# JunFenngZhi/YOLO-Fastest-and-Embedded-deployment

Hardware: AMD Instinct MI355X
Metric: frames/sec end-to-end (model forward + decode + per-class NMS), 320x256 batch=256 per GPU (higher is better)
Workload: dtype f32; 1 GPU; YOLO-Fastest 320x256 batch=256 fp32 per GPU, synthetic uniform-u8 frames (BASELINE.json configs[1]); global_batch=256, weights=yolo_fastest_256x320_epoch28.pth, kmax=64, chunk=0, in_flight=2, lanes=1, branches=0, world_size=1, parallelism=single GPU

## Files before the change

### yolo-fastest-and-embedded-deployment_amd/csrc/yf_mres_kernels.hip

```cpp
#include <hip/hip_runtime.h>
#include <math.h>
#include <stdint.h>

#include "yf_kernels.h"


namespace yf {



typedef float f32x4 __attribute__((ext_vector_type(4)));
typedef float f32x2 __attribute__((ext_vector_type(2)));
__device__ __forceinline__ float relu_bits(float x) { return __int_as_float(max(__float_as_int(x), 0)); }

template <int NT2>
__device__ __forceinline__ void mres_project_f32(float (&d)[4], const float (&w2f)[4][NT2], f32x4 (&acc)[NT2])
{
#pragma unroll
    for (int j = 0; j < 4; ++j) d[j] = relu_bits(d[j]);
    __builtin_amdgcn_sched_barrier(0);
#pragma unroll
    for (int j = 0; j < 4; ++j)
#pragma unroll
        for (int nt = 0; nt < NT2; ++nt) acc[nt] = __builtin_amdgcn_mfma_f32_16x16x4f32(w2f[j][nt], d[j], acc[nt], 0, 0, 0);
}

__host__ __device__ constexpr int mres_epl(int mtr, int s = 1) { return mtr * 16 + (s == 2 ? 1 : 0); }
__host__ __device__ constexpr int mres_ksteps(int K) { return (K / 16) * 4 + ((K % 16) ? 2 : 0); }
__host__ __device__ constexpr int mres_chunk_floats(int cin, int cout, int wmode = WM_F32)
{
    return wmode != WM_F32 ? (wmode == WM_F16X3 ? 2 : 1) * ((mres_ksteps(cin) + 3) / 4) * 128 + 16 + 9 * 16 + 16 +
                                 (wmode == WM_F16X3 ? 2 : 1) * ((cout + 15) / 16) * 128
                           : mres_ksteps(cin) * 64 + 16 + 9 * 16 + 16 + 4 * ((cout + 15) / 16) * 64;
}

template <int CIN, int S, int RW, int NRP, int MTR, int XP, int WFLOATS, int NTHR, typename T>
__device__ __forceinline__ void mres_stage(const MresArgs& a, int n, int oy0, int ox0, float* X, float* WL)
{
    constexpr int C4 = CIN / 4, NX = MTR * 16 * C4, NXI = (NX + NTHR - 1) / NTHR, NW4 = WFLOATS / 4, NWI = (NW4 + NTHR - 1) / NTHR;
    const T* __restrict__ src = reinterpret_cast<const T*>(a.in) + (long)n * a.H * a.W * CIN;
    float4 wv[NWI], xv[NXI];
#pragma unroll
    for (int i = 0; i < NWI; ++i) {
        const int idx = threadIdx.x + i * NTHR;
        wv[i] = float4(*reinterpret_cast<const float4*>(a.wp + 4 * (idx < NW4 ? idx : NW4 - 1)));
    }
#pragma unroll
    for (int i = 0; i < NXI; ++i) {
        const int idx = threadIdx.x + i * NTHR;
        const int rp = idx / C4, c4 = idx - rp * C4;
        const int ry = rp / RW, rx = rp - ry * RW;
        const int iy = oy0 * S - 1 + ry, ix = ox0 * S - 1 + rx;
        const bool ok = rp < NRP && iy >= 0 && iy < a.H && ix >= 0 && ix < a.W;
        xv[i] = ld4<T>(src + (ok ? (iy * a.W + ix) * CIN + c4 * 4 : 0));
        if (!ok) xv[i] = make_float4(0.f, 0.f, 0.f, 0.f);
    }
#pragma unroll
    for (int i = 0; i < NWI; ++i) {
        const int idx = threadIdx.x + i * NTHR;
        if (idx < NW4) *reinterpret_cast<float4*>(&WL[4 * idx]) = wv[i];
    }
#pragma unroll
    for (int i = 0; i < NXI; ++i) {
        const int idx = threadIdx.x + i * NTHR;
        const int rp = idx / C4, c4 = idx - rp * C4;
        if (idx < NX) *reinterpret_cast<float4*>(&X[rp * XP + c4 * 4]) = xv[i];
    }
}

__host__ __device__ constexpr bool mres_writes_expansion(int cin, int cexp, int cout, int s) { return cin == 24 && cexp == 136 && cout == 48 && s == 2; }
__host__ __device__ constexpr bool mres_relu_out(int cin, int cexp, int cout, int s) { return mres_writes_expansion(cin, cexp, cout, s); }

template <int TH, int TW, int RW, int S>
__device__ __forceinline__ void mres_out_px(int mo, int r, int& oy, int& ox)
{
    if constexpr (S == 1 && RW % 16 == 6 && TW % 2 == 0 && TH % 8 == 0) {
        const int rb = mo / (TW / 2), cp = mo - rb * (TW / 2);
        oy = rb * 8 + (r >> 1);
        ox = cp * 2 + (r & 1);
    } else if constexpr (S == 1 && RW % 16 == 12 && TW == 10 && TH == 8) {
        if (mo < 4) { oy = (mo >> 1) * 4 + (r >> 2); ox = (mo & 1) * 4 + (r & 3); }
        else { oy = r >> 1; ox = 8 + (r & 1); }
    } else {
        const int op = mo * 16 + r;
        oy = op / TW;
        ox = op - oy * TW;
    }
}

template <int CIN, int CEXP, int COUT, bool RES, int S, int TH, int TW, int NWAVE, typename T>
__global__ void __launch_bounds__(NWAVE * 64) mres_kernel(MresArgs a)
{
    constexpr int RH = (TH - 1) * S + 3, RW = (TW - 1) * S + 3, NRP = RH * RW;
    constexpr int MTR = (NRP + 15) / 16, MTO = (TH * TW) / 16;
    constexpr int MTRW = (MTR + NWAVE - 1) / NWAVE, MTOW = (MTO + NWAVE - 1) / NWAVE;
    constexpr bool EVEN_R = MTR % NWAVE == 0, EVEN_O = MTO % NWAVE == 0;
    constexpr bool WEXP = mres_writes_expansion(CIN, CEXP, COUT, S);
    constexpr int XP = CIN + 4;
    constexpr int EPL = mres_epl(MTR, S);
    constexpr bool X3 = is_x3<T>::value;
    constexpr bool H16 = sizeof(T) == 2 || X3;
    constexpr int WM = X3 ? 2 : 1;
    constexpr int KS1 = mres_ksteps(CIN), NB1 = CIN / 16, NT2 = (COUT + 15) / 16, NCH = (CEXP + 15) / 16;
    constexpr int NK1 = (KS1 + 3) / 4;
    constexpr int OFF_B1 = H16 ? WM * NK1 * 128 : KS1 * 64, OFF_WD = OFF_B1 + 16, OFF_BD = OFF_WD + 144, OFF_W2 = OFF_BD + 16;
    constexpr int CHUNK = OFF_W2 + (H16 ? WM * NT2 * 128 : 4 * NT2 * 64);
    static_assert((TH * TW) % 16 == 0 && CIN % 8 == 0 && COUT % 4 == 0, "shape");
    static_assert(!RES || (CIN == COUT && S == 1), "residual needs same shape");
    static_assert(CHUNK == mres_chunk_floats(CIN, COUT, wmode_of<T>()), "pack layout");
    static_assert(MTRW <= 32, "in-image mask bits");
    extern __shared__ __attribute__((aligned(16))) float mres_smem[];
    float* X = mres_smem;
    float* E = mres_smem + MTR * 16 * XP;
    float* WL = E + 16 * EPL;
    constexpr int WFLOATS = (NCH * CHUNK + COUT + 3) & ~3;

    const int b = xcd_tile(blockIdx.x, gridDim.x);
    const int tx = b % a.tiles_x, ty = (b / a.tiles_x) % a.tiles_y, n = b / (a.tiles_x * a.tiles_y);
    const int oy0 = ty * TH, ox0 = tx * TW;
    const int Ho = a.H / S, Wo = a.W / S;
    const int wave = __builtin_amdgcn_readfirstlane((int)(threadIdx.x >> 6));
    const int lane = threadIdx.x & 63, r = lane & 15, q = lane >> 4;

    mres_stage<CIN, S, RW, NRP, MTR, XP, WFLOATS, NWAVE * 64, T>(a, n, oy0, ox0, X, WL);
    __syncthreads();

    float a1[MTRW][KS1];
    unsigned inmask = 0;
    int eoff[MTRW];
#pragma unroll
    for (int i = 0; i < MTRW; ++i) {
        const int mt = wave + i * NWAVE;
        const int row = (mt < MTR ? mt : 0) * 16 + r;
#pragma unroll
        for (int kb = 0; kb < NB1; ++kb) {
            const float4 t = *reinterpret_cast<const float4*>(&X[row * XP + kb * 16 + 4 * q]);
            a1[i][kb * 4 + 0] = t.x; a1[i][kb * 4 + 1] = t.y; a1[i][kb * 4 + 2] = t.z; a1[i][kb * 4 + 3] = t.w;
        }
        if constexpr (CIN % 16 != 0) {
            const float2 t = *reinterpret_cast<const float2*>(&X[row * XP + NB1 * 16 + 2 * q]);
            a1[i][NB1 * 4 + 0] = t.x; a1[i][NB1 * 4 + 1] = t.y;
        }
        {
            const int rp = mt * 16 + r;
            const int ry = rp / RW, rx = rp - ry * RW;
            const int iy = oy0 * S - 1 + ry, ix = ox0 * S - 1 + rx;
            if (mt < MTR && rp < NRP && iy >= 0 && iy < a.H && ix >= 0 && ix < a.W) inmask |= 1u << i;
            eoff[i] = (inmask >> i & 1) && ry > 0 && rx > 0 ? (iy * a.W + ix) * CEXP + 4 * q : -1;
        }
    }
    f16x4 a1h[X3 ? MTRW : 1][NK1], a1l[X3 ? MTRW : 1][NK1];
    if constexpr (X3) {
#pragma unroll
        for (int i = 0; i < MTRW; ++i)
#pragma unroll
            for (int s = 0; s < NK1; ++s)
                split_f16x4(a1[i][4 * s], a1[i][4 * s + 1], 4 * s + 2 < KS1 ? a1[i][(4 * s + 2) % KS1] : 0.f,
                            4 * s + 3 < KS1 ? a1[i][(4 * s + 3) % KS1] : 0.f, a1h[i][s], a1l[i][s]);
    }
    f32x4 acc[MTOW][NT2];
    int rp0[MTOW];
#pragma unroll
    for (int i = 0; i < MTOW; ++i) {
#pragma unroll
        for (int nt = 0; nt < NT2; ++nt) acc[i][nt] = f32x4{0.f, 0.f, 0.f, 0.f};
        const int mo = wave + i * NWAVE;
        int oy, ox;
        mres_out_px<TH, TW, RW, S>(mo < MTO ? mo : 0, r, oy, ox);
        rp0[i] = (oy * S + 1) * RW + ox * S + 1;
    }

#pragma unroll 1
    for (int c = 0; c < NCH; ++c) {
        const float* wc = WL + c * CHUNK;
        float w1f[KS1];
        f16x4 w1h[NK1], w1l[X3 ? NK1 : 1];
        if constexpr (H16) {
#pragma unroll
            for (int s = 0; s < NK1; ++s) w1h[s] = reinterpret_cast<const f16x4*>(wc)[s * 64 + lane];
            if constexpr (X3) {
#pragma unroll
                for (int s = 0; s < NK1; ++s) w1l[s] = reinterpret_cast<const f16x4*>(wc)[(NK1 + s) * 64 + lane];
            }
        } else {
#pragma unroll
            for (int s = 0; s < KS1; ++s) w1f[s] = wc[s * 64 + lane];
        }
        const float4 b1 = *reinterpret_cast<const float4*>(wc + OFF_B1 + 4 * q);
        float4 wd[9];
#pragma unroll
        for (int t = 0; t < 9; ++t) wd[t] = *reinterpret_cast<const float4*>(wc + OFF_WD + t * 16 + 4 * q);
        const float4 bd = *reinterpret_cast<const float4*>(wc + OFF_BD + 4 * q);
        float w2f[4][NT2];
        f16x4 w2h[NT2], w2l[X3 ? NT2 : 1];
        if constexpr (H16) {
#pragma unroll
            for (int nt = 0; nt < NT2; ++nt) w2h[nt] = reinterpret_cast<const f16x4*>(wc + OFF_W2)[nt * 64 + lane];
            if constexpr (X3) {
#pragma unroll
                for (int nt = 0; nt < NT2; ++nt) w2l[nt] = reinterpret_cast<const f16x4*>(wc + OFF_W2)[(NT2 + nt) * 64 + lane];
            }
        } else {
#pragma unroll
            for (int j = 0; j < 4; ++j)
#pragma unroll
                for (int nt = 0; nt < NT2; ++nt) w2f[j][nt] = wc[OFF_W2 + (j * NT2 + nt) * 64 + lane];
        }

#pragma unroll
        for (int i = 0; i < MTRW; ++i) {
            const int mt = wave + i * NWAVE;
            if (EVEN_R || i < MTRW - 1 || mt < MTR) {
                f32x4 cf = f32x4{b1.x, b1.y, b1.z, b1.w};
                if constexpr (X3) {
#pragma unroll
                    for (int s = 0; s < NK1; ++s) {
                        cf = __builtin_amdgcn_mfma_f32_16x16x16f16(w1l[s], a1h[i][s], cf, 0, 0, 0);
                        cf = __builtin_amdgcn_mfma_f32_16x16x16f16(w1h[s], a1l[i][s], cf, 0, 0, 0);
                    }
#pragma unroll
                    for (int s = 0; s < NK1; ++s) cf = __builtin_amdgcn_mfma_f32_16x16x16f16(w1h[s], a1h[i][s], cf, 0, 0, 0);
                } else if constexpr (H16) {
#pragma unroll
                    for (int s = 0; s < NK1; ++s) {
                        const f16x4 ah = f16x4{(half_t)a1[i][4 * s], (half_t)a1[i][4 * s + 1], 4 * s + 2 < KS1 ? (half_t)a1[i][(4 * s + 2) % KS1] : (half_t)0.f,
                                               4 * s + 3 < KS1 ? (half_t)a1[i][(4 * s + 3) % KS1] : (half_t)0.f};
                        cf = __builtin_amdgcn_mfma_f32_16x16x16f16(w1h[s], ah, cf, 0, 0, 0);
                    }
                } else {
#pragma unroll
                    for (int s = 0; s < KS1; ++s) cf = __builtin_amdgcn_mfma_f32_16x16x4f32(w1f[s], a1[i][s], cf, 0, 0, 0);
                }
                const float lim = (inmask >> i) & 1 ? __builtin_inff() : 0.f;
                const float4 ev = make_float4(__builtin_amdgcn_fmed3f(cf[0], 0.f, lim), __builtin_amdgcn_fmed3f(cf[1], 0.f, lim),
                                              __builtin_amdgcn_fmed3f(cf[2], 0.f, lim), __builtin_amdgcn_fmed3f(cf[3], 0.f, lim));
                *reinterpret_cast<float4*>(E + (q * EPL + mt * 16 + r) * 4) = ev;
                if constexpr (WEXP)
                    if (eoff[i] >= 0 && c * 16 + 4 * q < CEXP)
                        st4<T>(reinterpret_cast<T*>(a.out_exp) + (long)n * a.H * a.W * CEXP + eoff[i] + c * 16, ev);
            }
        }
        __syncthreads();
#pragma unroll
        for (int i = 0; i < MTOW; ++i) {
            const int mo = wave + i * NWAVE;
            if (EVEN_O || i < MTOW - 1 || mo < MTO) {
                const float4* e = reinterpret_cast<const float4*>(E) + q * EPL + rp0[i];
                float d[4] = {bd.x, bd.y, bd.z, bd.w};
                constexpr bool BATCH9 = CEXP > 32;
                float4 v9[9];
                if constexpr (BATCH9) {
#pragma unroll
                    for (int t = 0; t < 9; ++t) v9[t] = e[(t / 3 - 1) * RW + (t % 3 - 1)];
                    __builtin_amdgcn_sched_barrier(0);
                }
                f32x2 dl = {d[0], d[1]}, dh2 = {d[2], d[3]};
#pragma unroll
                for (int t = 0; t < 9; ++t) {
                    float4 v;
                    if constexpr (BATCH9) v = v9[t]; else v = e[(t / 3 - 1) * RW + (t % 3 - 1)];
                    const float4 w = wd[t];
                    dl = __builtin_elementwise_fma(f32x2{v.x, v.y}, f32x2{w.x, w.y}, dl);
                    dh2 = __builtin_elementwise_fma(f32x2{v.z, v.w}, f32x2{w.z, w.w}, dh2);
                }
                d[0] = dl[0]; d[1] = dl[1]; d[2] = dh2[0]; d[3] = dh2[1];
                if constexpr (X3) {
                    f16x4 dh, dl;
                    split_f16x4(relu_bits(d[0]), relu_bits(d[1]), relu_bits(d[2]), relu_bits(d[3]), dh, dl);
#pragma unroll
                    for (int nt = 0; nt < NT2; ++nt) acc[i][nt] = __builtin_amdgcn_mfma_f32_16x16x16f16(w2l[nt], dh, acc[i][nt], 0, 0, 0);
#pragma unroll
                    for (int nt = 0; nt < NT2; ++nt) acc[i][nt] = __builtin_amdgcn_mfma_f32_16x16x16f16(w2h[nt], dl, acc[i][nt], 0, 0, 0);
#pragma unroll
                    for (int nt = 0; nt < NT2; ++nt) acc[i][nt] = __builtin_amdgcn_mfma_f32_16x16x16f16(w2h[nt], dh, acc[i][nt], 0, 0, 0);
                } else if constexpr (H16) {
                    const f16x4 dh = f16x4{(half_t)fmaxf(d[0], 0.f), (half_t)fmaxf(d[1], 0.f), (half_t)fmaxf(d[2], 0.f), (half_t)fmaxf(d[3], 0.f)};
#pragma unroll
                    for (int nt = 0; nt < NT2; ++nt) acc[i][nt] = __builtin_amdgcn_mfma_f32_16x16x16f16(w2h[nt], dh, acc[i][nt], 0, 0, 0);
                } else {
                    mres_project_f32<NT2>(d, w2f, acc[i]);
                }
            }
        }
        __syncthreads();
    }

    const float* b2 = WL + NCH * CHUNK;
#pragma unroll
    for (int i = 0; i < MTOW; ++i) {
        const int mo = wave + i * NWAVE;
        if (!EVEN_O && i == MTOW - 1 && mo >= MTO) continue;
        int oy, ox;
        mres_out_px<TH, TW, RW, S>(mo, r, oy, ox);
        const int gy = oy0 + oy, gx = ox0 + ox;
        if (gy >= Ho || gx >= Wo) continue;
#pragma unroll
        for (int nt = 0; nt < NT2; ++nt) {
            const int col = nt * 16 + 4 * q;
            if (col >= COUT) continue;
            const float4 bias = *reinterpret_cast<const float4*>(b2 + col);
            float4 v = make_float4(acc[i][nt][0] + bias.x, acc[i][nt][1] + bias.y, acc[i][nt][2] + bias.z, acc[i][nt][3] + bias.w);
            if constexpr (RES) {
                const float4 x = *reinterpret_cast<const float4*>(&X[((oy + 1) * RW + ox + 1) * XP + col]);
                v.x += x.x; v.y += x.y; v.z += x.z; v.w += x.w;
            }
            if constexpr (mres_relu_out(CIN, CEXP, COUT, S)) v = make_float4(fmaxf(v.x, 0.f), fmaxf(v.y, 0.f), fmaxf(v.z, 0.f), fmaxf(v.w, 0.f));
            st4<T>(reinterpret_cast<T*>(a.out) + (((long)n * Ho + gy) * Wo + gx) * COUT + col, v);
        }
    }
}


template <int K, int NOUT>
struct MresPostFrag { float w[mres_ksteps(K)]; float4 bias; };

template <int K, int NOUT, int NWAVE>
__device__ __forceinline__ void mres_post_fetch(const float* __restrict__ pw, int wave, int lane, MresPostFrag<K, NOUT>& f)
{
    constexpr int KS = mres_ksteps(K), NT = NOUT / 16;
    static_assert(K % 16 == 0 && NOUT % 16 == 0 && NWAVE >= NT, "post conv shape");
    const int nt = wave % NT;
#pragma unroll
    for (int s = 0; s < KS; ++s) f.w[s] = pw[(s * NT + nt) * 64 + lane];
    f.bias = *reinterpret_cast<const float4*>(pw + KS * NT * 64 + nt * 16 + 4 * (lane >> 4));
}

template <int K, int NOUT, int TH, int TW, int RW, int XP, int NWAVE, typename T>
__device__ __forceinline__ void mres_post_conv(const float* X, const MresPostFrag<K, NOUT>& f, T* __restrict__ out, int wave, int lane,
                                               int n, int oy0, int ox0, int H, int W)
{
    constexpr int NB = K / 16, NT = NOUT / 16, MTO = (TH * TW) / 16, NG = NWAVE / NT;
    const int r = lane & 15, q = lane >> 4;
    const int nt = wave % NT, g = wave / NT;
    if (g >= NG) return;
#pragma unroll 1
    for (int mt = g; mt < MTO; mt += NG) {
        const int p = mt * 16 + r, oy = p / TW, ox = p - oy * TW;
        const float* xr = X + ((oy + 1) * RW + ox + 1) * XP + 4 * q;
        float4 av[NB];
#pragma unroll
        for (int kb = 0; kb < NB; ++kb) av[kb] = *reinterpret_cast<const float4*>(xr + kb * 16);
        f32x4 acc = f32x4{0.f, 0.f, 0.f, 0.f};
#pragma unroll
        for (int kb = 0; kb < NB; ++kb)
#pragma unroll
            for (int j = 0; j < 4; ++j) acc = __builtin_amdgcn_mfma_f32_16x16x4f32(f.w[kb * 4 + j], ((const float*)&av[kb])[j], acc, 0, 0, 0);
        const int gy = oy0 + oy, gx = ox0 + ox;
        if (gy >= H || gx >= W) continue;
        const float4 v = make_float4(fmaxf(acc[0] + f.bias.x, 0.f), fmaxf(acc[1] + f.bias.y, 0.f), fmaxf(acc[2] + f.bias.z, 0.f),
                                     fmaxf(acc[3] + f.bias.w, 0.f));
        st4<T>(out + (((long)n * H + gy) * W + gx) * NOUT + nt * 16 + 4 * q, v);
    }
}

template <int CIN, int CEXP, int COUT, bool RES, int TH, int TW, int NWP, int NWC, typename T, int POSTN = 0, bool FRAME = false, int CPP = 1>
__global__ void __launch_bounds__((NWP + NWC) * 64) mres_pc_kernel(MresArgs a)
{
    constexpr int NWAVE = NWP + NWC;
    constexpr int RH = TH + 2, RW = TW + 2, NRP = RH * RW;
    constexpr int MTR = (NRP + 15) / 16, MTO = (TH * TW) / 16;
    constexpr int MTP = FRAME ? MTO : MTR;
    constexpr int MTRW = (MTP + NWP - 1) / NWP, MTOW = (MTO + NWC - 1) / NWC;
    constexpr int XP = CIN + 4;
    constexpr int EPL = mres_epl(MTR);
    constexpr bool X3 = is_x3<T>::value;
    constexpr bool H16 = sizeof(T) == 2 || X3;
    constexpr int WM = X3 ? 2 : 1;
    constexpr int KS1 = mres_ksteps(CIN), NB1 = CIN / 16, NT2 = (COUT + 15) / 16, NCH = (CEXP + 15) / 16;
    constexpr int NK1 = (KS1 + 3) / 4;
    constexpr int OFF_B1 = H16 ? WM * NK1 * 128 : KS1 * 64, OFF_WD = OFF_B1 + 16, OFF_BD = OFF_WD + 144, OFF_W2 = OFF_BD + 16;
    constexpr int CHUNK = OFF_W2 + (H16 ? WM * NT2 * 128 : 4 * NT2 * 64);
    static_assert((TH * TW) % 16 == 0 && CIN % 8 == 0 && COUT % 4 == 0, "shape");
    static_assert(CHUNK == mres_chunk_floats(CIN, COUT, wmode_of<T>()), "pack layout");
    static_assert(!RES || CIN == COUT, "residual needs same shape");
    static_assert(MTRW * 4 <= 64, "in-image mask bits");
    extern __shared__ __attribute__((aligned(16))) float mres_smem[];
    float* X = mres_smem;
    float* E = mres_smem + MTR * 16 * XP;
    float* WL = E + 2 * CPP * 16 * EPL;
    constexpr int NPH = ((CEXP + 15) / 16) / CPP;
    static_assert(((CEXP + 15) / 16) % CPP == 0, "chunks per phase must divide the chunk count");
    constexpr int WFLOATS = (NCH * CHUNK + COUT + 3) & ~3;
    constexpr bool PSUM = !H16 && CIN == 48 && CEXP == 224 && COUT == 48;

    const int b = xcd_tile(blockIdx.x, gridDim.x);
    const int tx = b % a.tiles_x, ty = (b / a.tiles_x) % a.tiles_y, n = b / (a.tiles_x * a.tiles_y);
    const int oy0 = ty * TH, ox0 = tx * TW;
    const int wave = __builtin_amdgcn_readfirstlane((int)(threadIdx.x >> 6));
    const int lane = threadIdx.x & 63, r = lane & 15, q = lane >> 4;
// ... 134 lines not shown
            mres_out_px<TH, TW, RW, 1>(mo < MTO ? mo : 0, r, oy, ox);
            rp0[i] = (oy + 1) * RW + ox + 1;
        }
#pragma unroll 1
      for (int blk = 0; blk < nblk; ++blk) {
        f32x4 acc[MTOW][NT2];
#pragma unroll
        for (int i = 0; i < MTOW; ++i)
#pragma unroll
            for (int nt = 0; nt < NT2; ++nt) acc[i][nt] = f32x4{0.f, 0.f, 0.f, 0.f};
#pragma unroll 1
        for (int ph = 0; ph <= NPH; ++ph) {
#pragma unroll
            for (int u = 0; u < CPP; ++u)
            if (ph >= 1) {
                const int s1 = (ph - 1) * CPP + u;
                const float* wc = WL + s1 * CHUNK;
                const float* Eb = E + (((ph - 1) & 1) * CPP + u) * 16 * EPL;
                float4 wd[9];
#pragma unroll
                for (int t = 0; t < 9; ++t) wd[t] = *reinterpret_cast<const float4*>(wc + OFF_WD + t * 16 + 4 * q);
                const float4 bd = *reinterpret_cast<const float4*>(wc + OFF_BD + 4 * q);
                float w2f[4][NT2];
                f16x4 w2h[NT2], w2l[X3 ? NT2 : 1];
                if constexpr (H16) {
#pragma unroll
                    for (int nt = 0; nt < NT2; ++nt) w2h[nt] = reinterpret_cast<const f16x4*>(wc + OFF_W2)[nt * 64 + lane];
                    if constexpr (X3) {
#pragma unroll
                        for (int nt = 0; nt < NT2; ++nt) w2l[nt] = reinterpret_cast<const f16x4*>(wc + OFF_W2)[(NT2 + nt) * 64 + lane];
                    }
                } else {
#pragma unroll
                    for (int j = 0; j < 4; ++j)
#pragma unroll
                        for (int nt = 0; nt < NT2; ++nt) w2f[j][nt] = wc[OFF_W2 + (j * NT2 + nt) * 64 + lane];
                }
#pragma unroll
                for (int i = 0; i < MTOW; ++i) {
                    const int mo = cw + i * NWC;
                    if (i < MTOW - 1 || mo < MTO) {
                        const float4* e = reinterpret_cast<const float4*>(Eb) + q * EPL + rp0[i];
                        float d[4] = {bd.x, bd.y, bd.z, bd.w};
                        float4 v9[9];
#pragma unroll
                        for (int t = 0; t < 9; ++t) v9[t] = e[(t / 3 - 1) * RW + (t % 3 - 1)];
                        __builtin_amdgcn_sched_barrier(0);
                        f32x2 dl = {d[0], d[1]}, dh2 = {d[2], d[3]};
#pragma unroll
                        for (int t = 0; t < 9; ++t) {
                            const float4 v = v9[t], w = wd[t];
                            dl = __builtin_elementwise_fma(f32x2{v.x, v.y}, f32x2{w.x, w.y}, dl);
                            dh2 = __builtin_elementwise_fma(f32x2{v.z, v.w}, f32x2{w.z, w.w}, dh2);
                        }
                        d[0] = dl[0]; d[1] = dl[1]; d[2] = dh2[0]; d[3] = dh2[1];
                        if constexpr (X3) {
                            f16x4 dh, dl;
                            split_f16x4(relu_bits(d[0]), relu_bits(d[1]), relu_bits(d[2]), relu_bits(d[3]), dh, dl);
#pragma unroll
                            for (int nt = 0; nt < NT2; ++nt) acc[i][nt] = __builtin_amdgcn_mfma_f32_16x16x16f16(w2l[nt], dh, acc[i][nt], 0, 0, 0);
#pragma unroll
                            for (int nt = 0; nt < NT2; ++nt) acc[i][nt] = __builtin_amdgcn_mfma_f32_16x16x16f16(w2h[nt], dl, acc[i][nt], 0, 0, 0);
#pragma unroll
                            for (int nt = 0; nt < NT2; ++nt) acc[i][nt] = __builtin_amdgcn_mfma_f32_16x16x16f16(w2h[nt], dh, acc[i][nt], 0, 0, 0);
                        } else if constexpr (H16) {
                            const f16x4 dh = f16x4{(half_t)fmaxf(d[0], 0.f), (half_t)fmaxf(d[1], 0.f), (half_t)fmaxf(d[2], 0.f),
                                                   (half_t)fmaxf(d[3], 0.f)};
#pragma unroll
                            for (int nt = 0; nt < NT2; ++nt)
                                acc[i][nt] = __builtin_amdgcn_mfma_f32_16x16x16f16(w2h[nt], dh, acc[i][nt], 0, 0, 0);
                        } else if constexpr (PSUM) {
                            f32x4 part[NT2];
#pragma unroll
                            for (int nt = 0; nt < NT2; ++nt) part[nt] = f32x4{0.f, 0.f, 0.f, 0.f};
                            mres_project_f32<NT2>(d, w2f, part);
#pragma unroll
                            for (int nt = 0; nt < NT2; ++nt) acc[i][nt] += part[nt];
                        } else {
                            mres_project_f32<NT2>(d, w2f, acc[i]);
                        }
                    }
                }
            }
            __syncthreads();
        }
        const bool last = blk + 1 == nblk;
        const float* b2 = WL + NCH * CHUNK;
#pragma unroll
        for (int i = 0; i < MTOW; ++i) {
            const int mo = cw + i * NWC;
            if (i == MTOW - 1 && mo >= MTO) continue;
            int oy, ox;
            mres_out_px<TH, TW, RW, 1>(mo, r, oy, ox);
            const int gy = oy0 + oy, gx = ox0 + ox;
            if (gy >= a.H || gx >= a.W) continue;
#pragma unroll
            for (int nt = 0; nt < NT2; ++nt) {
                const int col = nt * 16 + 4 * q;
                if (col >= COUT) continue;
                const float4 bias = *reinterpret_cast<const float4*>(b2 + col);
                float4 v = make_float4(acc[i][nt][0] + bias.x, acc[i][nt][1] + bias.y, acc[i][nt][2] + bias.z, acc[i][nt][3] + bias.w);
                float* xr = &X[((oy + 1) * RW + ox + 1) * XP + col];
                if constexpr (RES) {
                    const float4 x = *reinterpret_cast<const float4*>(xr);
                    v.x += x.x; v.y += x.y; v.z += x.z; v.w += x.w;
                }
                if (last && POSTN == 0) st4<T>(reinterpret_cast<T*>(a.out) + (((long)n * a.H + gy) * a.W + gx) * COUT + col, v);
                else *reinterpret_cast<float4*>(xr) = v;
            }
        }
        if (!last) {
            __syncthreads();
            __syncthreads();
        }
      }
      if constexpr (POSTN > 0) {
          MresPostFrag<COUT, POSTN> pf;
          mres_post_fetch<COUT, POSTN, NWAVE>(a.post_w, wave, lane, pf);
          __syncthreads();
          mres_post_conv<COUT, POSTN, TH, TW, RW, XP, NWAVE, T>(X, pf, reinterpret_cast<T*>(a.post_out), wave, lane, n, oy0, ox0, a.H, a.W);
      }
    }
}

template <int CIN, int CEXP, int COUT, bool RES, int TH, int TW, int NWP, int NWC, typename T, int POSTN = 0, bool FRAME = false>
static int launch_mres_pc_t(MresArgs a, int N, hipStream_t s)
{
    constexpr int CPP = 1;
    a.tiles_y = (a.H + TH - 1) / TH;
    a.tiles_x = (a.W + TW - 1) / TW;
    if constexpr (!FRAME) {
        if (a.tiles_y == 1 && a.tiles_x == 1) return launch_mres_pc_t<CIN, CEXP, COUT, RES, TH, TW, NWP, NWC, T, POSTN, true>(a, N, s);
    }
    constexpr int MTR = ((TH + 2) * (TW + 2) + 15) / 16;
    constexpr size_t lds = ((size_t)MTR * 16 * (CIN + 4) + 2 * CPP * 16 * mres_epl(MTR) +
                            ((((CEXP + 15) / 16) * mres_chunk_floats(CIN, COUT, wmode_of<T>()) + COUT + 3) & ~3)) * sizeof(float);
    static_assert(lds <= 160 * 1024, "LDS");
    static bool attr_done[YF_MAX_DEVICES] = {};
    const int dev = current_device();
    if (dev < 0) return -2;
    if (lds > 64 * 1024 && !attr_done[dev]) {
        if (hipFuncSetAttribute(reinterpret_cast<const void*>(mres_pc_kernel<CIN, CEXP, COUT, RES, TH, TW, NWP, NWC, T, POSTN, FRAME, CPP>),
                                hipFuncAttributeMaxDynamicSharedMemorySize, (int)lds) != hipSuccess)
            return -2;
        attr_done[dev] = true;
    }
    if (a.nblk > 1 && (a.tiles_y != 1 || a.tiles_x != 1 || !RES)) return -4;
    if ((POSTN > 0) != (a.post_w != nullptr) || (POSTN > 0 && !a.post_out)) return -5;
    hipLaunchKernelGGL((mres_pc_kernel<CIN, CEXP, COUT, RES, TH, TW, NWP, NWC, T, POSTN, FRAME, CPP>), dim3((unsigned)(N * a.tiles_y * a.tiles_x)),
                       dim3((NWP + NWC) * 64), lds, s, a);
    return 0;
}

template <int CIN, int CEXP, int COUT, bool RES, int S, int TH, int TW, int NWAVE, typename T>
static int launch_mres_t(MresArgs a, int N, hipStream_t s)
{
    a.tiles_y = (a.H / S + TH - 1) / TH;
    a.tiles_x = (a.W / S + TW - 1) / TW;
    if (mres_writes_expansion(CIN, CEXP, COUT, S) && !a.out_exp) return -3;
    if (a.nblk > 1) return -4;
    constexpr int MTR = (((TH - 1) * S + 3) * ((TW - 1) * S + 3) + 15) / 16;
    constexpr size_t lds = ((size_t)MTR * 16 * (CIN + 4) + 16 * mres_epl(MTR, S) +
                            ((((CEXP + 15) / 16) * mres_chunk_floats(CIN, COUT, wmode_of<T>()) + COUT + 3) & ~3)) * sizeof(float);
    static_assert(lds <= 160 * 1024, "LDS");
    static bool attr_done[YF_MAX_DEVICES] = {};
    const int dev = current_device();
    if (dev < 0) return -2;
    if (lds > 64 * 1024 && !attr_done[dev]) {
        if (hipFuncSetAttribute(reinterpret_cast<const void*>(mres_kernel<CIN, CEXP, COUT, RES, S, TH, TW, NWAVE, T>),
                                hipFuncAttributeMaxDynamicSharedMemorySize, (int)lds) != hipSuccess)
            return -2;
        attr_done[dev] = true;
    }
    hipLaunchKernelGGL((mres_kernel<CIN, CEXP, COUT, RES, S, TH, TW, NWAVE, T>), dim3((unsigned)(N * a.tiles_y * a.tiles_x)),
                       dim3(NWAVE * 64), lds, s, a);
    return 0;
}

constexpr int RES5_NWP = 3, RES5_NWC = 5;
#define YF_MRES_SHAPES(MR)                                                            \
    MR(8, 48, 8, true, 1, 16, 20, 0, 8)              \
    MR(8, 48, 16, false, 1, 16, 20, 0, 8)            \
    MR(16, 96, 16, true, 1, 16, 20, 0, 8)            \
    MR(16, 96, 24, false, 2, 8, 10, 0, 8)       \
    MR(8, 32, 8, false, 2, 8, 10, 0, 8)         \
    MR(24, 136, 48, false, 2, 8, 10, 0, 8)   \
    MR(24, 136, 24, true, 1, 16, 20, 4, 8)           \
    MR(48, 224, 48, true, 1, 8, 10, RES5_NWP, RES5_NWC)

template <int CIN, int CEXP, int COUT, bool RES, int S, int TH, int TW, int NWP, int NW, typename T>
static int launch_mres_any(const MresArgs& a, int N, hipStream_t s)
{
    if constexpr (NWP == 0) return launch_mres_t<CIN, CEXP, COUT, RES, S, TH, TW, NW, T>(a, N, s);
    else { static_assert(S == 1, "producer/consumer kernel: stride 1 only"); return launch_mres_pc_t<CIN, CEXP, COUT, RES, TH, TW, NWP, NW, T>(a, N, s); }
}

bool mres_has_post(int cin, int cexp, int cout, int postn) { return cin == 48 && cexp == 224 && cout == 48 && postn == 96; }
size_t mres_post_packed_floats(int cout, int postn) { return (size_t)mres_ksteps(cout) * (postn / 16) * 64 + postn; }

struct EsplitArgs {
    const float* in;
    const float* wp;
    long wstride;
    float* out;
    const float* post_w;
    float* post_out;
    float* xbuf;
    float* slab;
    int nblk, k, n_frames;
};

template <int CIN, int CEXP, int TH, int TW, int POSTN>
__global__ void __launch_bounds__(((TH * TW) / 16) * 64) mres_esplit_kernel(EsplitArgs a)
{
    constexpr int COUT = CIN, NPX = TH * TW, MT = NPX / 16, NWAVE = MT, RH = TH + 2, RW = TW + 2, XP = CIN + 4;
    constexpr int KS1 = mres_ksteps(CIN), NB1 = CIN / 16, NT2 = COUT / 16, NCH = (CEXP + 15) / 16;
    constexpr int OFF_B1 = KS1 * 64, OFF_WD = OFF_B1 + 16, OFF_BD = OFF_WD + 144, OFF_W2 = OFF_BD + 16, CHUNK = OFF_W2 + 4 * NT2 * 64;
    constexpr int EPL = ((RH * RW + 15) / 16) * 16;
    static_assert(NPX % 16 == 0 && CIN % 16 == 0 && CHUNK == mres_chunk_floats(CIN, COUT, WM_F32), "shape / pack layout");
    __shared__ __attribute__((aligned(16))) float X[NPX * XP];
    __shared__ __attribute__((aligned(16))) float E[4 * EPL * 4];
    const int n = blockIdx.x / NCH, g = blockIdx.x - n * NCH;
    const int lane = threadIdx.x & 63, r = lane & 15, q = lane >> 4;
    const int wave = __builtin_amdgcn_readfirstlane((int)(threadIdx.x >> 6));
    const int k = a.k;
    constexpr int C4 = CIN / 4, NX4 = NPX * C4, NTHR = NWAVE * 64;
    const long fr = (long)NPX * CIN;
    if (k == 0) {
        for (int i = threadIdx.x; i < NX4; i += NTHR) {
            const int px = i / C4, c4 = i - px * C4;
            *reinterpret_cast<float4*>(&X[px * XP + c4 * 4]) = *reinterpret_cast<const float4*>(a.in + n * fr + (long)px * CIN + c4 * 4);
        }
    } else {
        const float* xprev = (k == 1 ? a.in : a.xbuf + ((long)((k - 1) & 1) * a.n_frames) * fr) + n * fr;
        const float* sl = a.slab + (((long)((k - 1) & 1) * a.n_frames + n) * NCH) * fr;
        const float* b2 = a.wp + (long)(k - 1) * a.wstride + NCH * CHUNK;
        float* xnext = a.xbuf + ((long)(k & 1) * a.n_frames + n) * fr;
        for (int i = threadIdx.x; i < NX4; i += NTHR) {
            const int px = i / C4, c4 = i - px * C4;
            const long o = (long)px * CIN + c4 * 4;
            float4 v = *reinterpret_cast<const float4*>(sl + o);
#pragma unroll
            for (int c = 1; c < NCH; ++c) {
                const float4 t = *reinterpret_cast<const float4*>(sl + c * fr + o);
                v.x += t.x; v.y += t.y; v.z += t.z; v.w += t.w;
            }
            const float4 bb = *reinterpret_cast<const float4*>(b2 + c4 * 4);
            const float4 xx = *reinterpret_cast<const float4*>(xprev + o);
            v.x = (v.x + bb.x) + xx.x; v.y = (v.y + bb.y) + xx.y; v.z = (v.z + bb.z) + xx.z; v.w = (v.w + bb.w) + xx.w;
            *reinterpret_cast<float4*>(&X[px * XP + c4 * 4]) = v;
            if (g == 0 && k < a.nblk) *reinterpret_cast<float4*>(xnext + o) = v;
            if (g == 0 && k == a.nblk && a.out) *reinterpret_cast<float4*>(a.out + n * fr + o) = v;
        }
    }
    for (int i = threadIdx.x; i < 4 * EPL; i += NTHR) reinterpret_cast<float4*>(E)[i] = make_float4(0.f, 0.f, 0.f, 0.f);
    __syncthreads();
    const int p = wave * 16 + r, py = p / TW, pxx = p - py * TW;
    const int rp = (py + 1) * RW + pxx + 1;
    if (k == a.nblk) {
        if constexpr (POSTN > 0) {
            constexpr int NTP = POSTN / 16;
            if (!a.post_w || g >= NTP) return;
            const float* pw = a.post_w;
            float4 av[NB1];
#pragma unroll
            for (int kb = 0; kb < NB1; ++kb) av[kb] = *reinterpret_cast<const float4*>(&X[p * XP + kb * 16 + 4 * q]);
            f32x4 acc = f32x4{0.f, 0.f, 0.f, 0.f};
#pragma unroll
            for (int kb = 0; kb < NB1; ++kb)
#pragma unroll
                for (int j = 0; j < 4; ++j)
                    acc = __builtin_amdgcn_mfma_f32_16x16x4f32(pw[((kb * 4 + j) * NTP + g) * 64 + lane], ((const float*)&av[kb])[j], acc, 0, 0, 0);
            const float4 bias = *reinterpret_cast<const float4*>(pw + KS1 * NTP * 64 + g * 16 + 4 * q);
            *reinterpret_cast<float4*>(a.post_out + ((long)n * NPX + p) * POSTN + g * 16 + 4 * q) =
                make_float4(fmaxf(acc[0] + bias.x, 0.f), fmaxf(acc[1] + bias.y, 0.f), fmaxf(acc[2] + bias.z, 0.f), fmaxf(acc[3] + bias.w, 0.f));
        }
        return;
    }
    const float* wc = a.wp + (long)k * a.wstride + g * CHUNK;
    float a1[KS1], w1f[KS1];
#pragma unroll
    for (int kb = 0; kb < NB1; ++kb) {
        const float4 t = *reinterpret_cast<const float4*>(&X[p * XP + kb * 16 + 4 * q]);
        a1[kb * 4 + 0] = t.x; a1[kb * 4 + 1] = t.y; a1[kb * 4 + 2] = t.z; a1[kb * 4 + 3] = t.w;
    }
#pragma unroll
    for (int s = 0; s < KS1; ++s) w1f[s] = wc[s * 64 + lane];
    const float4 b1 = *reinterpret_cast<const float4*>(wc + OFF_B1 + 4 * q);
    float4 wd[9];
#pragma unroll
    for (int t = 0; t < 9; ++t) wd[t] = *reinterpret_cast<const float4*>(wc + OFF_WD + t * 16 + 4 * q);
    const float4 bd = *reinterpret_cast<const float4*>(wc + OFF_BD + 4 * q);
    float w2f[4][NT2];
#pragma unroll
    for (int j = 0; j < 4; ++j)
#pragma unroll
        for (int nt = 0; nt < NT2; ++nt) w2f[j][nt] = wc[OFF_W2 + (j * NT2 + nt) * 64 + lane];
    f32x4 cf = f32x4{b1.x, b1.y, b1.z, b1.w};
#pragma unroll
    for (int s = 0; s < KS1; ++s) cf = __builtin_amdgcn_mfma_f32_16x16x4f32(w1f[s], a1[s], cf, 0, 0, 0);
    *reinterpret_cast<float4*>(E + (q * EPL + rp) * 4) = make_float4(fmaxf(cf[0], 0.f), fmaxf(cf[1], 0.f), fmaxf(cf[2], 0.f), fmaxf(cf[3], 0.f));
    __syncthreads();
    const float4* e = reinterpret_cast<const float4*>(E) + q * EPL + rp;
    float d[4] = {bd.x, bd.y, bd.z, bd.w};
#pragma unroll
    for (int t = 0; t < 9; ++t) {
        const float4 v = e[(t / 3 - 1) * RW + (t % 3 - 1)];
        d[0] = fmaf(v.x, wd[t].x, d[0]); d[1] = fmaf(v.y, wd[t].y, d[1]); d[2] = fmaf(v.z, wd[t].z, d[2]); d[3] = fmaf(v.w, wd[t].w, d[3]);
    }
    f32x4 acc[NT2];
#pragma unroll
    for (int nt = 0; nt < NT2; ++nt) acc[nt] = f32x4{0.f, 0.f, 0.f, 0.f};
#pragma unroll
    for (int j = 0; j < 4; ++j) {
        const float dj = relu_bits(d[j]);
#pragma unroll
        for (int nt = 0; nt < NT2; ++nt) acc[nt] = __builtin_amdgcn_mfma_f32_16x16x4f32(w2f[j][nt], dj, acc[nt], 0, 0, 0);
    }
    float* so = a.slab + ((((long)(k & 1) * a.n_frames + n) * NCH + g) * NPX + p) * CIN + 4 * q;
#pragma unroll
    for (int nt = 0; nt < NT2; ++nt) *reinterpret_cast<float4*>(so + nt * 16) = make_float4(acc[nt][0], acc[nt][1], acc[nt][2], acc[nt][3]);
}

enum { ESPLIT_MAX_FRAMES = 9 };
size_t mres_esplit_scratch_floats() { return (size_t)ESPLIT_MAX_FRAMES * (2 + 2 * 14) * 80 * 48; }
static bool mres_esplit_ok(const MresArgs& a, int N, int dtype)
{
    return dtype == DT_F32 && a.esplit && a.nblk > 1 && a.H == 8 && a.W == 10 && N <= ESPLIT_MAX_FRAMES;
}
// ... 157 lines not shown
```

Measured before the change: 309,000 frames/s.

## Compact expansion rows to in-image pixels to skip padded halo MFMA work

Adds an in-image mode to the inverted-residual kernel: instead of running the 1x1 expansion MFMA over the whole halo region (including out-of-image padding), each wave processes a compacted list of only in-image halo pixels, mapped back to region coordinates with a reciprocal divide. The per-wave row-tile count is chosen at compile time from the worst-case in-image span, and the host checks whether all tiles fit under it. The expansion buffer is pre-zeroed when a tile has padding. This removes MFMA work for padded rows on border tiles, in exchange for extra index arithmetic, scattered LDS writes and a zero-fill pass. It only pays off where the smaller tile count covers every tile.

```diff
diff --git a/yolo-fastest-and-embedded-deployment_amd/csrc/yf_mres_kernels.hip b/yolo-fastest-and-embedded-deployment_amd/csrc/yf_mres_kernels.hip
--- a/yolo-fastest-and-embedded-deployment_amd/csrc/yf_mres_kernels.hip
+++ b/yolo-fastest-and-embedded-deployment_amd/csrc/yf_mres_kernels.hip
@@ -88,13 +88,34 @@
     }
 }
 
-template <int CIN, int CEXP, int COUT, bool RES, int S, int TH, int TW, int NWAVE, typename T>
+__host__ __device__ inline void mres_span(int o0, int S, int R, int n, int& lo, int& hi)
+{
+    const int first = o0 * S - 1;
+    lo = first < 0 ? -first : 0;
+    hi = n - first < R ? n - first : R;
+}
+static int mres_max_inimage(int H, int W, int S, int TH, int TW)
+{
+    const int RH = (TH - 1) * S + 3, RW = (TW - 1) * S + 3;
+    int most = 0;
+    for (int ty = 0; ty * TH < H / S; ++ty)
+        for (int tx = 0; tx * TW < W / S; ++tx) {
+            int y0, y1, x0, x1;
+            mres_span(ty * TH, S, RH, H, y0, y1);
+            mres_span(tx * TW, S, RW, W, x0, x1);
+            if ((y1 - y0) * (x1 - x0) > most) most = (y1 - y0) * (x1 - x0);
+        }
+    return most;
+}
+
+template <int CIN, int CEXP, int COUT, bool RES, int S, int TH, int TW, int NWAVE, typename T, int XS = 0>
 __global__ void __launch_bounds__(NWAVE * 64) mres_kernel(MresArgs a)
 {
     constexpr int RH = (TH - 1) * S + 3, RW = (TW - 1) * S + 3, NRP = RH * RW;
     constexpr int MTR = (NRP + 15) / 16, MTO = (TH * TW) / 16;
-    constexpr int MTRW = (MTR + NWAVE - 1) / NWAVE, MTOW = (MTO + NWAVE - 1) / NWAVE;
-    constexpr bool EVEN_R = MTR % NWAVE == 0, EVEN_O = MTO % NWAVE == 0;
+    constexpr bool INIMG = XS > 0;
+    constexpr int MTRW = INIMG ? XS : (MTR + NWAVE - 1) / NWAVE, MTOW = (MTO + NWAVE - 1) / NWAVE;
+    constexpr bool EVEN_R = !INIMG && MTR % NWAVE == 0, EVEN_O = MTO % NWAVE == 0;
     constexpr bool WEXP = mres_writes_expansion(CIN, CEXP, COUT, S);
     constexpr int XP = CIN + 4;
     constexpr int EPL = mres_epl(MTR, S);
@@ -109,6 +130,7 @@
     static_assert(!RES || (CIN == COUT && S == 1), "residual needs same shape");
     static_assert(CHUNK == mres_chunk_floats(CIN, COUT, wmode_of<T>()), "pack layout");
     static_assert(MTRW <= 32, "in-image mask bits");
+    static_assert(MTRW * NWAVE * 16 * ((TW - 1) * S + 3) < (1 << 20), "in-image form: k / rwi by multiplication");
     extern __shared__ __attribute__((aligned(16))) float mres_smem[];
     float* X = mres_smem;
     float* E = mres_smem + MTR * 16 * XP;
@@ -123,15 +145,31 @@
     const int lane = threadIdx.x & 63, r = lane & 15, q = lane >> 4;
 
     mres_stage<CIN, S, RW, NRP, MTR, XP, WFLOATS, NWAVE * 64, T>(a, n, oy0, ox0, X, WL);
+    int ry0 = 0, ry1 = RH, rx0 = 0, rx1 = RW;
+    if constexpr (INIMG) { mres_span(oy0, S, RH, a.H, ry0, ry1); mres_span(ox0, S, RW, a.W, rx0, rx1); }
+    const int rwi = rx1 - rx0, nin = (ry1 - ry0) * rwi, nexp = (nin + 15) >> 4;
+    const unsigned rwi_rcp = ((1u << 20) + rwi - 1) / rwi;
+    if constexpr (INIMG) {
+        if (nin < NRP)
+            for (int i = threadIdx.x; i < 4 * EPL; i += NWAVE * 64) reinterpret_cast<float4*>(E)[i] = make_float4(0.f, 0.f, 0.f, 0.f);
+    }
     __syncthreads();
 
     float a1[MTRW][KS1];
     unsigned inmask = 0;
     int eoff[MTRW];
+    int erec[INIMG ? MTRW : 1];
 #pragma unroll
     for (int i = 0; i < MTRW; ++i) {
         const int mt = wave + i * NWAVE;
-        const int row = (mt < MTR ? mt : 0) * 16 + r;
+        int row = (mt < MTR ? mt : 0) * 16 + r, ry_i = 0, rx_i = 0;
+        if constexpr (INIMG) {
+            const int k = min(mt * 16 + r, nin - 1);
+            const int ky = (int)((unsigned)k * rwi_rcp >> 20);
+            ry_i = ry0 + ky; rx_i = rx0 + k - ky * rwi;
+            row = ry_i * RW + rx_i;
+            erec[i] = q * EPL + row;
+        }
 #pragma unroll
         for (int kb = 0; kb < NB1; ++kb) {
             const float4 t = *reinterpret_cast<const float4*>(&X[row * XP + kb * 16 + 4 * q]);
@@ -141,7 +179,9 @@
             const float2 t = *reinterpret_cast<const float2*>(&X[row * XP + NB1 * 16 + 2 * q]);
             a1[i][NB1 * 4 + 0] = t.x; a1[i][NB1 * 4 + 1] = t.y;
         }
-        {
+        if constexpr (INIMG) {
+            eoff[i] = mt * 16 + r < nin && ry_i > 0 && rx_i > 0 ? ((oy0 * S - 1 + ry_i) * a.W + ox0 * S - 1 + rx_i) * CEXP + 4 * q : -1;
+        } else {
             const int rp = mt * 16 + r;
             const int ry = rp / RW, rx = rp - ry * RW;
             const int iy = oy0 * S - 1 + ry, ix = ox0 * S - 1 + rx;
@@ -169,6 +209,8 @@
         mres_out_px<TH, TW, RW, S>(mo < MTO ? mo : 0, r, oy, ox);
         rp0[i] = (oy * S + 1) * RW + ox * S + 1;
     }
+    float lim_in = __builtin_inff();
+    if constexpr (INIMG) asm volatile("" : "+s"(lim_in));
 
 #pragma unroll 1
     for (int c = 0; c < NCH; ++c) {
@@ -210,7 +252,7 @@
 #pragma unroll
         for (int i = 0; i < MTRW; ++i) {
             const int mt = wave + i * NWAVE;
-            if (EVEN_R || i < MTRW - 1 || mt < MTR) {
+            if (EVEN_R || i < MTRW - 1 || mt < (INIMG ? nexp : MTR)) {
                 f32x4 cf = f32x4{b1.x, b1.y, b1.z, b1.w};
                 if constexpr (X3) {
 #pragma unroll
@@ -231,10 +273,11 @@
 #pragma unroll
                     for (int s = 0; s < KS1; ++s) cf = __builtin_amdgcn_mfma_f32_16x16x4f32(w1f[s], a1[i][s], cf, 0, 0, 0);
                 }
-                const float lim = (inmask >> i) & 1 ? __builtin_inff() : 0.f;
+                const float lim = INIMG ? lim_in : (inmask >> i) & 1 ? __builtin_inff() : 0.f;
                 const float4 ev = make_float4(__builtin_amdgcn_fmed3f(cf[0], 0.f, lim), __builtin_amdgcn_fmed3f(cf[1], 0.f, lim),
                                               __builtin_amdgcn_fmed3f(cf[2], 0.f, lim), __builtin_amdgcn_fmed3f(cf[3], 0.f, lim));
-                *reinterpret_cast<float4*>(E + (q * EPL + mt * 16 + r) * 4) = ev;
+                if constexpr (INIMG) reinterpret_cast<float4*>(E)[erec[i]] = ev;
+                else *reinterpret_cast<float4*>(E + (q * EPL + mt * 16 + r) * 4) = ev;
                 if constexpr (WEXP)
                     if (eoff[i] >= 0 && c * 16 + 4 * q < CEXP)
                         st4<T>(reinterpret_cast<T*>(a.out_exp) + (long)n * a.H * a.W * CEXP + eoff[i] + c * 16, ev);
@@ -675,8 +718,8 @@
     return 0;
 }
 
-template <int CIN, int CEXP, int COUT, bool RES, int S, int TH, int TW, int NWAVE, typename T>
-static int launch_mres_t(MresArgs a, int N, hipStream_t s)
+template <int CIN, int CEXP, int COUT, bool RES, int S, int TH, int TW, int NWAVE, typename T, int XS>
+static int launch_mres_x(MresArgs a, int N, hipStream_t s)
 {
     a.tiles_y = (a.H / S + TH - 1) / TH;
     a.tiles_x = (a.W / S + TW - 1) / TW;
@@ -690,14 +733,29 @@
     const int dev = current_device();
     if (dev < 0) return -2;
     if (lds > 64 * 1024 && !attr_done[dev]) {
-        if (hipFuncSetAttribute(reinterpret_cast<const void*>(mres_kernel<CIN, CEXP, COUT, RES, S, TH, TW, NWAVE, T>),
+        if (hipFuncSetAttribute(reinterpret_cast<const void*>(mres_kernel<CIN, CEXP, COUT, RES, S, TH, TW, NWAVE, T, XS>),
                                 hipFuncAttributeMaxDynamicSharedMemorySize, (int)lds) != hipSuccess)
             return -2;
         attr_done[dev] = true;
     }
-    hipLaunchKernelGGL((mres_kernel<CIN, CEXP, COUT, RES, S, TH, TW, NWAVE, T>), dim3((unsigned)(N * a.tiles_y * a.tiles_x)),
+    hipLaunchKernelGGL((mres_kernel<CIN, CEXP, COUT, RES, S, TH, TW, NWAVE, T, XS>), dim3((unsigned)(N * a.tiles_y * a.tiles_x)),
                        dim3(NWAVE * 64), lds, s, a);
     return 0;
+}
+
+template <int CIN, int CEXP, int COUT, bool RES, int S, int TH, int TW, int NWAVE, typename T>
+static int launch_mres_t(const MresArgs& a, int N, hipStream_t s)
+{
+    constexpr int RH = (TH - 1) * S + 3, RW = (TW - 1) * S + 3;
+    constexpr int XFULL = ((RH * RW + 15) / 16 + NWAVE - 1) / NWAVE;
+    constexpr int XEDGE = (((RH - 1) * RW > RH * (RW - 1) ? (RH - 1) * RW : RH * (RW - 1)) + 15) / 16;
+    constexpr int XBORDER = (XEDGE + NWAVE - 1) / NWAVE;
+    if constexpr (XBORDER < XFULL) {
+        if (mres_max_inimage(a.H, a.W, S, TH, TW) <= XBORDER * NWAVE * 16) return launch_mres_x<CIN, CEXP, COUT, RES, S, TH, TW, NWAVE, T, XBORDER>(a, N, s);
+        return launch_mres_x<CIN, CEXP, COUT, RES, S, TH, TW, NWAVE, T, 0>(a, N, s);
+    } else {
+        return launch_mres_x<CIN, CEXP, COUT, RES, S, TH, TW, NWAVE, T, XFULL>(a, N, s);
+    }
 }
 
 constexpr int RES5_NWP = 3, RES5_NWC = 5;
```

New measurement: 312,900 frames/s (median of 6 runs). +1.3%, better.
